# Vegeta2020/SE-SSD

Hardware: AMD Instinct MI355X
Metric: KITTI frames/sec (voxelize->backbone->head->NMS) (higher is better)
Workload: dtype f32

## Files before the change

### se-ssd_amd/csrc/dense_wino_sk.hip

```cpp
#include <cstdlib>
#include "common.hpp"
#include "bf16_split.hpp"

namespace {

using f32x16 = __attribute__((ext_vector_type(16))) float;
using f32x4v = __attribute__((ext_vector_type(4))) float;
using f32x2v = __attribute__((ext_vector_type(2))) float;
typedef unsigned int u32x4g __attribute__((__vector_size__(16)));
typedef __bf16 bf16x8 __attribute__((ext_vector_type(8)));
typedef __bf16 bf16x2 __attribute__((ext_vector_type(2)));

typedef __amdgpu_buffer_rsrc_t rsrc_t;
__device__ __forceinline__ rsrc_t make_rsrc(const void* base, unsigned bytes) {
  return __builtin_amdgcn_make_buffer_rsrc(const_cast<void*>(base), (short)0, (int)bytes, 0x00020000);
}
#define SESSD_OOB 0x80000000u
#define SESSD_LDS_BARRIER() asm volatile("s_waitcnt lgkmcnt(0)\n\ts_barrier" ::: "memory")
#define SESSD_SYSTEM_SCOPE 17

__device__ __forceinline__ float sadd(float a, float b) {
  float r;
  asm volatile("v_add_f32 %0, %1, %2" : "=v"(r) : "v"(a), "v"(b));
  return r;
}

using sessd::pk_bf16;
using sessd::split3_pk;

struct WinoArgs {
  const float* in;
  const float* upk;
  float* out;
  const float* scale;
  const float* shift;
  const float* residual;
  float* scratch;
  unsigned* counters;
  int cin, hin, win, cout, relu;
  int tw, ntiles, tblocks, ngroups, rpu, total_rounds;
  int bper;
  int ss_stride;
  long long upk_stride;
  const int* tile_list;
  const int* n_list;
  int list_cap, min_rounds, batch;
};

template <int NW, int CBN, int VAR = 0, bool LIST = false, bool SPLIT = false>
__global__ __launch_bounds__(NW * 64, 8 / NW) void conv3x3s1_winograd_sk_kernel(WinoArgs A) {
  constexpr int XW = 16 / NW;
  static_assert(XW * CBN == 8, "8 accumulators per wave");
  static_assert(!SPLIT || (NW == 8 && VAR == 0), "the split main loop is written for 8 waves (a round = one K = 16 MFMA)");
  constexpr int VBUF_S = 3 * 16 * 64 * 4;
  constexpr int NT = NW * 64;
  constexpr unsigned WSTEP = NW * 2u * 32u * 32u;
  constexpr int VBUF = NW * 1024;
  constexpr int SLOT = CBN * 32 * 32 * 4;
  constexpr int NPT = 1024 / NT;
  constexpr int RING = NW;
  __shared__ __attribute__((aligned(16))) float lds[SPLIT ? 2 * VBUF_S : 16384];
  __shared__ int s_last, s_pend;
  const int tid = threadIdx.x, lane = tid & 63;
  const int wave = __builtin_amdgcn_readfirstlane(tid >> 6);
  const int j = lane & 31, h = lane >> 5;
  int G = gridDim.x;
  long long R = A.total_rounds;
  int n_list = 0;
  if constexpr (LIST) {
    n_list = __builtin_amdgcn_readfirstlane(min(A.n_list[0], A.list_cap));
    R = (long long)((n_list + 31) >> 5) * A.ngroups * A.rpu;
    if (R == 0) return;
    if (A.min_rounds < 0) {
      const long long U = R / A.rpu;
      long long g = U / (-A.min_rounds);
      g = g < 1 ? 1 : (g > G ? G : g);
      G = (int)g;
      if ((int)blockIdx.x >= G) return;
    } else {
      long long g = R / A.min_rounds;
      g = g < 1 ? 1 : (g > G ? G : g);
      G = (int)(g >= 8 ? (g & ~7LL) : g);
      if ((G & 7) ? ((int)blockIdx.x >= G) : ((int)(blockIdx.x >> 3) >= (G >> 3))) return;
    }
  }
  const bool whole_units = LIST && A.min_rounds < 0;
  const int w = (whole_units || (G & 7)) ? (int)blockIdx.x : (int)((blockIdx.x & 7) * (G >> 3) + (blockIdx.x >> 3));
  int r = whole_units ? (int)((long long)w * (R / A.rpu) / G) * A.rpu : (int)((long long)w * R / G);
  const int r_stop = whole_units ? (int)((long long)(w + 1) * (R / A.rpu) / G) * A.rpu : (int)((long long)(w + 1) * R / G);
  const int in_plane = A.hin * A.win;
  const size_t out_plane = (size_t)in_plane;
  const unsigned xstep = 2u * (unsigned)in_plane * 4u;
  const unsigned wo = (unsigned)(((wave * 2 + h) * 32 + j) * 32);

  int pend_state = 0, pend_u = 0, pend_first = 0, pend_last = 0, pend_tbase = 0, pend_mbase = 0, pend_b = 0;
#define SESSD_SK_SIGNAL()                                                                          \
  {                                                                                                \
    __builtin_amdgcn_s_waitcnt(0);                                                                 \
    __syncthreads();                                                                               \
    if (tid == 0) {                                                                                \
      const unsigned old = __hip_atomic_fetch_add(A.counters + pend_u, 1u, __ATOMIC_RELAXED, __HIP_MEMORY_SCOPE_AGENT); \
      s_pend = (old == (unsigned)(pend_last - pend_first)) ? 1 : 0;                                \
    }                                                                                              \
    __syncthreads();                                                                               \
    pend_state = s_pend ? 2 : 0;                                                                   \
  }

#define SESSD_SK_FINALIZE(Y, CO, SC, SH)                                                            \
  if (tok && (CO) < e_cout) {                                                                       \
    _Pragma("unroll") for (int a = 0; a < 2; ++a) {                                                 \
      const size_t o = (size_t)(CO) * out_plane + pix + (size_t)a * e_win;                          \
      float v0 = fmaf((Y)[2 * a], (SC), (SH)), v1 = fmaf((Y)[2 * a + 1], (SC), (SH));              \
      if (e_relu) { v0 = fmaxf(v0, 0.f); v1 = fmaxf(v1, 0.f); }                                 \
      if (resb) { v0 += resb[o]; v1 += resb[o + 1]; }                                               \
      *reinterpret_cast<float2*>(outb + o) = make_float2(v0, v1);                                   \
    }                                                                                               \
  }
#define SESSD_SK_FINISH_PENDING()                                                                  \
  {                                                                                                \
    const __attribute__((address_space(4))) WinoArgs* Fp =                                         \
        (const __attribute__((address_space(4))) WinoArgs*)__builtin_amdgcn_kernarg_segment_ptr(); \
    asm volatile("" : "+s"(Fp));                                                                   \
    const int f_set = pend_b / Fp->bper;                                                           \
    const float* f_scale = Fp->scale ? Fp->scale + (size_t)f_set * Fp->ss_stride : nullptr;        \
    const float* f_shift = Fp->shift ? Fp->shift + (size_t)f_set * Fp->ss_stride : nullptr;        \
    const int e_cout = Fp->cout, e_relu = Fp->relu, e_win = Fp->win, f_tw = Fp->tw;                \
    const rsrc_t fr = make_rsrc(Fp->scratch, (unsigned)(2 * G) * SLOT * 4u);                       \
    float* outb = Fp->out + (size_t)pend_b * e_cout * out_plane;                                   \
    const float* resb = Fp->residual ? Fp->residual + (size_t)pend_b * e_cout * out_plane : nullptr; \
    const int tl = tid & 31, col0 = tid >> 5;                                                      \
    int tt = pend_tbase + tl;                                                                      \
    bool tok = tt < Fp->ntiles;                                                                    \
    size_t pix = 0;                                                                                \
    if constexpr (LIST) {                                                                          \
      const int fe = tt < n_list ? Fp->tile_list[tt] : -1;                                         \
      tok = fe >= 0;                                                                               \
      const int fb = tok ? fe / Fp->ntiles : 0;                                                    \
      tt = tok ? fe - fb * Fp->ntiles : 0;                                                         \
      pix = (size_t)fb * e_cout * out_plane;                                                       \
    }                                                                                              \
    const int oty = tok ? tt / f_tw : 0, otx = tok ? tt - (tt / f_tw) * f_tw : 0;                  \
    pix += (size_t)(2 * oty) * e_win + 2 * otx;                                                    \
    _Pragma("unroll 1") for (int cb = 0; cb < CBN; ++cb) {                                         \
      f32x4v ysum[NPT];                                                                            \
      _Pragma("unroll") for (int n = 0; n < NPT; ++n) ysum[n] = 0.f;                               \
      for (int wq = pend_first; wq <= pend_last; ++wq) {                                           \
        const unsigned slot = (unsigned)(2 * wq + (wq == pend_first ? 1 : 0)) * (unsigned)(SLOT * 4); \
        f32x4v p[NPT];                                                                             \
        _Pragma("unroll") for (int n = 0; n < NPT; ++n)                                            \
          p[n] = __builtin_bit_cast(f32x4v, __builtin_amdgcn_raw_buffer_load_b128(                 \
              fr, (int)(slot + (unsigned)(((cb * 32 + col0 + (NT / 32) * n) * 32 + tl) * 16)), 0, SESSD_SYSTEM_SCOPE)); \
        _Pragma("unroll") for (int n = 0; n < NPT; ++n) ysum[n] += p[n];                           \
      }                                                                                            \
      _Pragma("unroll") for (int n = 0; n < NPT; ++n) {                                            \
        const int co = pend_mbase + cb * 32 + col0 + (NT / 32) * n;                                \
        const float scv = (f_scale && co < e_cout) ? f_scale[co] : 1.f, shv = (f_shift && co < e_cout) ? f_shift[co] : 0.f; \
        const float z[4] = {ysum[n].x, ysum[n].y, ysum[n].z, ysum[n].w};                           \
        SESSD_SK_FINALIZE(z, co, scv, shv)                                                         \
      }                                                                                            \
    }                                                                                              \
    if (tid == 0) __hip_atomic_store(Fp->counters + pend_u, 0u, __ATOMIC_RELAXED, __HIP_MEMORY_SCOPE_AGENT); \
    pend_state = 0;                                                                                \
  }

  while (r < r_stop) {
    const int u = __builtin_amdgcn_readfirstlane(r / A.rpu);
    const int r0 = __builtin_amdgcn_readfirstlane(r - u * A.rpu);
    const int r1 = __builtin_amdgcn_readfirstlane(min(r_stop - u * A.rpu, A.rpu));
    r = u * A.rpu + r1;
    const int cg = __builtin_amdgcn_readfirstlane(u % A.ngroups), ub = u / A.ngroups;
    const int tb = LIST ? __builtin_amdgcn_readfirstlane(ub) : __builtin_amdgcn_readfirstlane(ub % A.tblocks);
    const int b = LIST ? 0 : __builtin_amdgcn_readfirstlane(ub / A.tblocks);
    const int t_base = tb * 32, m_base = cg * (CBN * 32);
    const rsrc_t xr = LIST ? make_rsrc(A.in, (unsigned)A.batch * (unsigned)A.cin * (unsigned)in_plane * 4u)
                           : make_rsrc(A.in + (size_t)b * A.cin * in_plane, (unsigned)A.cin * in_plane * 4u);
    const int wset = LIST ? 0 : __builtin_amdgcn_readfirstlane(b / A.bper);
    const rsrc_t wr = make_rsrc(A.upk + (size_t)wset * A.upk_stride + (size_t)cg * (A.cin >> 1) * (WSTEP / 4), (unsigned)(A.cin >> 1) * WSTEP);

    int t = t_base + j;
    bool tlive = t < A.ntiles;
    unsigned img_off = 0;
    if constexpr (LIST) {
      const int e = t < n_list ? A.tile_list[t] : -1;
      tlive = e >= 0;
      const int bl = tlive ? e / A.ntiles : 0;
      t = tlive ? e - bl * A.ntiles : 0;
      img_off = (unsigned)bl * (unsigned)A.cin * (unsigned)in_plane * 4u;
    }
    const int ty = tlive ? t / A.tw : 0, tx = tlive ? t - (t / A.tw) * A.tw : 0;
    const int y0 = 2 * ty - 1, x0 = 2 * tx - 1;
    unsigned ro[4];
#pragma unroll
    for (int q = 0; q < 4; ++q) {
      const int y = y0 + q;
      ro[q] = (tlive && y >= 0 && y < A.hin) ? img_off + (unsigned)((h * in_plane + y * A.win + max(x0, 0)) * 4) : SESSD_OOB;
    }
    const bool mask_l = (tx == 0), mask_r = (tx == A.tw - 1);
    const bool edge = __builtin_amdgcn_ballot_w64(tlive && (mask_l || mask_r)) != 0;
    const int klast = r1 * NW - 1;

    f32x16 acc[XW][CBN];
#pragma unroll
    for (int x = 0; x < XW; ++x)
#pragma unroll
      for (int c = 0; c < CBN; ++c)
#pragma unroll
// ... 30 lines not shown
#define SESSD_SK_TRANSFORM(VOFF)                                                                   \
  {                                                                                                \
    if (edge) {                                                                                    \
      _Pragma("unroll") for (int q = 0; q < 4; ++q) {                                              \
        const f32x4v p = pr[q];                                                                    \
        pr[q].x = mask_l ? 0.f : p.x; pr[q].y = mask_l ? p.x : p.y;                                \
        pr[q].z = mask_l ? p.y : p.z; pr[q].w = mask_l ? p.z : (mask_r ? 0.f : p.w);               \
      }                                                                                            \
    }                                                                                              \
    f32x2v tl[4], tr[4];                                                                           \
    if constexpr (VAR & 1) {                                                                       \
      tl[0].x = sadd(pr[0].x, -pr[2].x); tl[0].y = sadd(pr[0].y, -pr[2].y); tr[0].x = sadd(pr[0].z, -pr[2].z); tr[0].y = sadd(pr[0].w, -pr[2].w); \
      tl[1].x = sadd(pr[1].x, pr[2].x); tl[1].y = sadd(pr[1].y, pr[2].y); tr[1].x = sadd(pr[1].z, pr[2].z); tr[1].y = sadd(pr[1].w, pr[2].w); \
      tl[2].x = sadd(pr[2].x, -pr[1].x); tl[2].y = sadd(pr[2].y, -pr[1].y); tr[2].x = sadd(pr[2].z, -pr[1].z); tr[2].y = sadd(pr[2].w, -pr[1].w); \
      tl[3].x = sadd(pr[1].x, -pr[3].x); tl[3].y = sadd(pr[1].y, -pr[3].y); tr[3].x = sadd(pr[1].z, -pr[3].z); tr[3].y = sadd(pr[1].w, -pr[3].w); \
    } else {                                                                                       \
    tl[0] = pr[0].xy - pr[2].xy; tr[0] = pr[0].zw - pr[2].zw;                                      \
    tl[1] = pr[1].xy + pr[2].xy; tr[1] = pr[1].zw + pr[2].zw;                                      \
    tl[2] = pr[2].xy - pr[1].xy; tr[2] = pr[2].zw - pr[1].zw;                                      \
    tl[3] = pr[1].xy - pr[3].xy; tr[3] = pr[1].zw - pr[3].zw;                                      \
    }                                                                                              \
    float* dst = &lds[(VOFF) + wave * 1024 + h * 32 + j];                                          \
    _Pragma("unroll") for (int a = 0; a < 4; ++a) {                                                \
      dst[(a * 4 + 0) * 64] = tl[a].x - tr[a].x;                                                   \
      dst[(a * 4 + 1) * 64] = tl[a].y + tr[a].x;                                                   \
      dst[(a * 4 + 2) * 64] = tr[a].x - tl[a].y;                                                   \
      dst[(a * 4 + 3) * 64] = tl[a].y - tr[a].y;                                                   \
    }                                                                                              \
  }
#define SESSD_SK_READV(P, KS, VOFF)                                                                \
  {                                                                                                \
    const float* vb = &lds[(VOFF) + (KS)*1024 + wave * (XW * 64) + h * 32 + j];                    \
    _Pragma("unroll") for (int x = 0; x < XW; ++x) bv[P][x] = vb[x * 64];                          \
  }
#define SESSD_SK_MMA(SET, P)                                                                       \
  {                                                                                                \
    if constexpr (VAR & 2) __builtin_amdgcn_s_setprio(3);                                          \
    _Pragma("unroll") for (int c = 0; c < CBN; ++c)                                                \
      _Pragma("unroll") for (int x = 0; x < XW; ++x)                                               \
        acc[x][c] = __builtin_amdgcn_mfma_f32_32x32x2f32(ua[SET][(c * XW + x) >> 2][(c * XW + x) & 3], bv[P][x], acc[x][c], 0, 0, 0); \
    if constexpr (VAR & 2) __builtin_amdgcn_s_setprio(0);                                          \
  }
#define SESSD_SK_STEP(KS)                                                                          \
  {                                                                                                \
    SESSD_SK_LOADU(((KS) + RING - 1) & (RING - 1), kg0 + (KS) + RING - 1)                          \
    if ((KS) < NW - 1) SESSD_SK_READV(((KS) + 1) & 1, (KS) + 1, voff)                              \
    __builtin_amdgcn_sched_barrier(0);                                                             \
    SESSD_SK_MMA((KS) & (RING - 1), (KS) & 1)                                                      \
    __builtin_amdgcn_sched_barrier(0);                                                             \
  }
#define SESSD_SK_ROUND()                                                                           \
  {                                                                                                \
    const int kg0 = rr * NW;                                                                       \
    SESSD_SK_LOADP(rr + 1)                                                                         \
    SESSD_SK_READV(0, 0, voff)                                                                     \
    __builtin_amdgcn_sched_barrier(0);                                                             \
    SESSD_SK_STEP(0)                                                                               \
    SESSD_SK_STEP(1)                                                                               \
    SESSD_SK_STEP(2)                                                                               \
    SESSD_SK_STEP(3)                                                                               \
    if constexpr (NW == 8) {                                                                       \
      SESSD_SK_STEP(4)                                                                             \
      SESSD_SK_STEP(5)                                                                             \
      SESSD_SK_STEP(6)                                                                             \
      SESSD_SK_STEP(7)                                                                             \
    }                                                                                              \
    SESSD_SK_TRANSFORM(voff ^ VBUF)                                                                \
    __syncthreads();                                                                               \
    voff ^= VBUF;                                                                                  \
    ++rr;                                                                                          \
  }
#define SESSD_SS_LOADP(ROUND)                                                                      \
  {                                                                                                \
    const unsigned xs = (unsigned)(min((ROUND), r1 - 1) * NW + wave) * xstep;                      \
    _Pragma("unroll") for (int c = 0; c < 2; ++c)                                                  \
      _Pragma("unroll") for (int q = 0; q < 3; ++q)                                                \
        ps[c][q] = __builtin_bit_cast(f32x4v, __builtin_amdgcn_raw_buffer_load_b128(xr, (int)rs[q], (int)(xs + c * (xstep >> 1)), 0)); \
  }
#define SESSD_SS_LOADU(SET, KG)                                                                    \
  {                                                                                                \
    const unsigned ws = (unsigned)min((KG), klast) * 3072u;                                        \
    _Pragma("unroll") for (int p = 0; p < 3; ++p)                                                  \
      us[SET][p] = __builtin_bit_cast(bf16x8, __builtin_amdgcn_raw_buffer_load_b128(wrs, (int)(wso + 1024u * p), (int)ws, 0)); \
  }
#define SESSD_SS_TRANSFORM(VOFF)                                                                   \
  {                                                                                                \
    if (edge) {                                                                                    \
      _Pragma("unroll") for (int c = 0; c < 2; ++c)                                                \
        _Pragma("unroll") for (int q = 0; q < 3; ++q) {                                            \
          const f32x4v p = ps[c][q];                                                               \
          ps[c][q].x = mask_l ? 0.f : p.x; ps[c][q].y = mask_l ? p.x : p.y;                        \
          ps[c][q].z = mask_l ? p.y : p.z; ps[c][q].w = mask_l ? p.z : (mask_r ? 0.f : p.w);       \
        }                                                                                          \
    }                                                                                              \
    float vt[2][8];                                                                                \
    _Pragma("unroll") for (int c = 0; c < 2; ++c) {                                                \
      const f32x4v ra = ps[c][0] - ps[c][1];                                                       \
      const f32x4v rb = ps[c][1] + (h ? -ps[c][2] : ps[c][2]);                                     \
      vt[c][0] = ra.x - ra.z; vt[c][1] = ra.y + ra.z; vt[c][2] = ra.z - ra.y; vt[c][3] = ra.y - ra.w; \
      vt[c][4] = rb.x - rb.z; vt[c][5] = rb.y + rb.z; vt[c][6] = rb.z - rb.y; vt[c][7] = rb.y - rb.w; \
    }                                                                                              \
    unsigned* dst = reinterpret_cast<unsigned*>(&lds[(VOFF) + ((8 * h) * 64 + (wave >> 2) * 32 + j) * 4 + (wave & 3)]); \
    _Pragma("unroll") for (int e = 0; e < 8; ++e) {                                                \
      unsigned t0, t1, t2;                                                                         \
      split3_pk(vt[0][e], vt[1][e], t0, t1, t2);                                                   \
      dst[e * 256] = t0; dst[(16 + e) * 256] = t1; dst[(32 + e) * 256] = t2;                       \
    }                                                                                              \
  }
#define SESSD_SS_READV(VOFF, X)                                                                    \
  {                                                                                                \
    _Pragma("unroll") for (int p = 0; p < 3; ++p)                                                  \
      bs[p] = __builtin_bit_cast(bf16x8, *static_cast<const u32x4g*>(__builtin_assume_aligned(                    \
          &lds[(VOFF) + ((p * 16 + wave * XW + (X)) * 64 + lane) * 4], 16)));                     \
  }
#define SESSD_SS_MMA(SET, S)                                                                       \
  {                                                                                                \
    f32x16 a_ = acc[(S) >> 2][(S) & 3];                                                            \
    a_ = __builtin_amdgcn_mfma_f32_32x32x16_bf16(us[SET][2], bs[0], a_, 0, 0, 0);                  \
    a_ = __builtin_amdgcn_mfma_f32_32x32x16_bf16(us[SET][1], bs[1], a_, 0, 0, 0);                  \
    a_ = __builtin_amdgcn_mfma_f32_32x32x16_bf16(us[SET][0], bs[2], a_, 0, 0, 0);                  \
    a_ = __builtin_amdgcn_mfma_f32_32x32x16_bf16(us[SET][1], bs[0], a_, 0, 0, 0);                  \
    a_ = __builtin_amdgcn_mfma_f32_32x32x16_bf16(us[SET][0], bs[1], a_, 0, 0, 0);                  \
    a_ = __builtin_amdgcn_mfma_f32_32x32x16_bf16(us[SET][0], bs[0], a_, 0, 0, 0);                  \
    acc[(S) >> 2][(S) & 3] = a_;                                                                   \
  }
#define SESSD_SS_STEP(KS)                                                                          \
  {                                                                                                \
    SESSD_SS_LOADU(((KS) + 3) & 3, kg0 + (KS) + 3)                                                 \
    __builtin_amdgcn_sched_barrier(0);                                                             \
    SESSD_SS_MMA((KS) & 3, KS)                                                                     \
    __builtin_amdgcn_sched_barrier(0);                                                             \
  }
#define SESSD_SS_ROUND()                                                                           \
  {                                                                                                \
    const int kg0 = rr * 8;                                                                        \
    SESSD_SS_READV(voff, 0)                                                                        \
    __builtin_amdgcn_sched_barrier(0);                                                             \
    SESSD_SS_STEP(0)                                                                               \
    SESSD_SS_STEP(1)                                                                               \
    SESSD_SS_STEP(2)                                                                               \
    SESSD_SS_STEP(3)                                                                               \
    SESSD_SS_LOADP(rr + 1)                                                                         \
    SESSD_SS_READV(voff, 1)                                                                        \
    __builtin_amdgcn_sched_barrier(0);                                                             \
    SESSD_SS_STEP(4)                                                                               \
    SESSD_SS_STEP(5)                                                                               \
    SESSD_SS_STEP(6)                                                                               \
    SESSD_SS_STEP(7)                                                                               \
    SESSD_SS_TRANSFORM(voff ^ VBUF_S)                                                              \
    __syncthreads();                                                                               \
    voff ^= VBUF_S;                                                                                \
    ++rr;                                                                                          \
  }

    if constexpr (SPLIT) {
      SESSD_SS_LOADP(r0)
      __builtin_amdgcn_sched_barrier(0);
#pragma unroll
      for (int s = 0; s < 3; ++s) {
        SESSD_SS_LOADU(s, r0 * 8 + s)
        __builtin_amdgcn_sched_barrier(0);
      }
      SESSD_SS_TRANSFORM(0)
    } else {
      SESSD_SK_LOADP(r0)
      __builtin_amdgcn_sched_barrier(0);
#pragma unroll
      for (int s = 0; s < RING - 1; ++s) {
        SESSD_SK_LOADU(s, r0 * NW + s)
        __builtin_amdgcn_sched_barrier(0);
      }
      SESSD_SK_TRANSFORM(0)
    }
    __syncthreads();
    if (pend_state == 1) {
      if (tid == 0) {
        const unsigned old = __hip_atomic_fetch_add(A.counters + pend_u, 1u, __ATOMIC_RELAXED, __HIP_MEMORY_SCOPE_AGENT);
        s_pend = (old == (unsigned)(pend_last - pend_first)) ? 1 : 0;
      }
      pend_state = 3;
    }
    int voff = 0;
    int rr = r0;
    if constexpr (SPLIT) {
      while (rr < r1) SESSD_SS_ROUND()
    } else {
      while (rr < r1) SESSD_SK_ROUND()
    }
#undef SESSD_SK_LOADP
#undef SESSD_SK_LOADU
#undef SESSD_SK_TRANSFORM
#undef SESSD_SK_READV
#undef SESSD_SK_MMA
#undef SESSD_SK_STEP
#undef SESSD_SK_ROUND
#undef SESSD_SS_LOADP
#undef SESSD_SS_LOADU
#undef SESSD_SS_TRANSFORM
#undef SESSD_SS_READV
#undef SESSD_SS_MMA
#undef SESSD_SS_STEP
#undef SESSD_SS_ROUND

    if (pend_state == 3) {
      SESSD_LDS_BARRIER();
      pend_state = s_pend ? 2 : 0;
    }
    const __attribute__((address_space(4))) WinoArgs* Ep =
        (const __attribute__((address_space(4))) WinoArgs*)__builtin_amdgcn_kernarg_segment_ptr();
    asm volatile("" : "+s"(Ep));
    const float* e_scale = Ep->scale ? Ep->scale + (size_t)wset * Ep->ss_stride : nullptr;
    const float* e_shift = Ep->shift ? Ep->shift + (size_t)wset * Ep->ss_stride : nullptr;
    const int e_cout = Ep->cout, e_relu = Ep->relu, e_win = Ep->win, e_tw = Ep->tw, e_ntiles = Ep->ntiles;
    unsigned* e_counter = Ep->counters + u;
    const rsrc_t sr = make_rsrc(Ep->scratch, (unsigned)(2 * G) * SLOT * 4u);
    const bool full = (r0 == 0 && r1 == Ep->rpu);
    float* outb = Ep->out + (size_t)b * e_cout * out_plane;
    const float* resb = Ep->residual ? Ep->residual + (size_t)b * e_cout * out_plane : nullptr;
    const int tl = tid & 31, col0 = tid >> 5;
    int tt = t_base + tl;
    bool tok = tt < e_ntiles;
    size_t pix = 0;
    if constexpr (LIST) {
      const int ee = tt < n_list ? Ep->tile_list[tt] : -1;
      tok = ee >= 0;
      const int eb = tok ? ee / e_ntiles : 0;
      tt = tok ? ee - eb * e_ntiles : 0;
      pix = (size_t)eb * e_cout * out_plane;
    }
    const int oty = tok ? tt / e_tw : 0, otx = tok ? tt - (tt / e_tw) * e_tw : 0;
    pix += (size_t)(2 * oty) * e_win + 2 * otx;
    const int w_first = (int)((((long long)u * Ep->rpu + 1) * G - 1) / R);
    const int w_last = (int)((((long long)u * Ep->rpu + Ep->rpu) * G - 1) / R);
    const unsigned my_slot = (unsigned)(2 * w + (r0 == 0 ? 1 : 0)) * (unsigned)(SLOT * 4);
    bool certain = false;
    unsigned oslot = 0;
    if (!full && w_last == w_first + 1) {
      if (tid == 0) s_last = __hip_atomic_load(e_counter, __ATOMIC_RELAXED, __HIP_MEMORY_SCOPE_AGENT) == 1u ? 1 : 0;
      __syncthreads();
      certain = s_last != 0;
      const int wq = (w == w_first) ? w_last : w_first;
      oslot = (unsigned)(2 * wq + (wq == w_first ? 1 : 0)) * (unsigned)(SLOT * 4);
    }
    const bool writes_out = full || certain;
    f32x4v onext[NPT];
    float scn[NPT], shn[NPT];
#define SESSD_SK_FETCH(CB)                                                                          \
  _Pragma("unroll") for (int n = 0; n < NPT; ++n) {                                                 \
    const int co_ = m_base + (CB)*32 + col0 + (NT / 32) * n;                                        \
    if (certain)                                                                                    \
      onext[n] = __builtin_bit_cast(                                                                \
          f32x4v, __builtin_amdgcn_raw_buffer_load_b128(                                            \
                      sr, (int)(oslot + (unsigned)((((CB)*32 + col0 + (NT / 32) * n) * 32 + tl) * 16)), 0, SESSD_SYSTEM_SCOPE)); \
    else                                                                                            \
      onext[n] = 0.f;                                                                               \
    scn[n] = (writes_out && e_scale && co_ < e_cout) ? e_scale[co_] : 1.f;                          \
    shn[n] = (writes_out && e_shift && co_ < e_cout) ? e_shift[co_] : 0.f;                          \
  }
    SESSD_SK_FETCH(0)
#pragma unroll
    for (int cb = 0; cb < CBN; ++cb) {
      if (cb) SESSD_LDS_BARRIER();
#pragma unroll
      for (int x = 0; x < XW; ++x)
#pragma unroll
        for (int q = 0; q < 16; ++q) {
          const int co = (q & 3) + 8 * (q >> 2) + 4 * h;
          lds[((wave * XW + x) * 32 + co) * 32 + j] = acc[x][cb][q];
        }
      f32x4v other[NPT];
      float sc[NPT], sh[NPT];
#pragma unroll
      for (int n = 0; n < NPT; ++n) { other[n] = onext[n]; sc[n] = scn[n]; sh[n] = shn[n]; }
      if (cb + 1 < CBN) { SESSD_SK_FETCH(cb + 1) }
      SESSD_LDS_BARRIER();
#pragma unroll
      for (int n = 0; n < NPT; ++n) {
        const int col = col0 + (NT / 32) * n;
        float m[16];
#pragma unroll
        for (int x = 0; x < 16; ++x) m[x] = lds[(x * 32 + col) * 32 + tl];
        float q0[4], q1[4];
#pragma unroll
        for (int c = 0; c < 4; ++c) {
          q0[c] = m[0 * 4 + c] + m[1 * 4 + c] + m[2 * 4 + c];
          q1[c] = m[1 * 4 + c] - m[2 * 4 + c] - m[3 * 4 + c];
        }
        float y[4];
        y[0] = q0[0] + q0[1] + q0[2]; y[1] = q0[1] - q0[2] - q0[3];
        y[2] = q1[0] + q1[1] + q1[2]; y[3] = q1[1] - q1[2] - q1[3];
        const int co = m_base + cb * 32 + col;
        if (full) {
          SESSD_SK_FINALIZE(y, co, sc[n], sh[n])
        } else if (certain) {
          const f32x4v o4 = other[n];
          const bool mine_first = (w == w_first);
          float z[4];
          z[0] = mine_first ? (0.f + y[0]) + o4.x : (0.f + o4.x) + y[0];
          z[1] = mine_first ? (0.f + y[1]) + o4.y : (0.f + o4.y) + y[1];
          z[2] = mine_first ? (0.f + y[2]) + o4.z : (0.f + o4.z) + y[2];
          z[3] = mine_first ? (0.f + y[3]) + o4.w : (0.f + o4.w) + y[3];
          SESSD_SK_FINALIZE(z, co, sc[n], sh[n])
        } else {
          f32x4v v;
          v.x = y[0]; v.y = y[1]; v.z = y[2]; v.w = y[3];
          __builtin_amdgcn_raw_buffer_store_b128(__builtin_bit_cast(u32x4g, v), sr,
                                                 (int)(my_slot + (unsigned)(((cb * 32 + col) * 32 + tl) * 16)), 0, SESSD_SYSTEM_SCOPE);
        }
      }
    }
    if (certain) {
      if (tid == 0) __hip_atomic_store(e_counter, 0u, __ATOMIC_RELAXED, __HIP_MEMORY_SCOPE_AGENT);
    } else if (!full) {
      if (pend_state == 2) SESSD_SK_FINISH_PENDING()
      pend_u = u; pend_first = w_first; pend_last = w_last; pend_tbase = t_base; pend_mbase = m_base; pend_b = b;
      pend_state = 1;
    }
#undef SESSD_SK_FETCH
    SESSD_LDS_BARRIER();
  }
  if (pend_state == 1) SESSD_SK_SIGNAL()
  if (pend_state == 2) SESSD_SK_FINISH_PENDING()
#undef SESSD_SK_FINALIZE
#undef SESSD_SK_SIGNAL
#undef SESSD_SK_FINISH_PENDING
}


template <int VAR = 0>
__global__ __launch_bounds__(256, 1) void conv3x3s1_winograd_rk_kernel(WinoArgs A) {
  constexpr int NW = 4, KR = 8, RING = 4;
  constexpr int NT = NW * 64;
  constexpr unsigned WSTEP = 4u * 2u * 32u * 16u * 4u;
  constexpr int VBUF = KR * 1024;
  constexpr int SLOT = 4 * 32 * 32 * 4;
  constexpr int NPT = 1024 / NT;
  __shared__ __attribute__((aligned(16))) float lds[2 * VBUF];
  __shared__ int s_last, s_pend;
  const int tid = threadIdx.x, lane = tid & 63;
  const int wave = __builtin_amdgcn_readfirstlane(tid >> 6);
  const int j = lane & 31, h = lane >> 5;
  const int G = gridDim.x;
  const int w = (G & 7) ? (int)blockIdx.x : (int)((blockIdx.x & 7) * (G >> 3) + (blockIdx.x >> 3));
  const long long R = A.total_rounds;
  int r = (int)((long long)w * R / G);
  const int r_stop = (int)((long long)(w + 1) * R / G);
  const int in_plane = A.hin * A.win;
  const size_t out_plane = (size_t)in_plane;
  const unsigned xstep = 2u * (unsigned)in_plane * 4u;
  const unsigned wo = (unsigned)(((wave * 2 + h) * 32 + j) * 64);

  int pend_state = 0, pend_u = 0, pend_first = 0, pend_last = 0, pend_tbase = 0, pend_mbase = 0, pend_b = 0;
#define SESSD_RK_SIGNAL()                                                                          \
  {                                                                                                \
    __builtin_amdgcn_s_waitcnt(0);                                                                 \
// ... 192 lines not shown
#undef SESSD_RK_READV
#undef SESSD_RK_MMA
#undef SESSD_RK_STEP
#undef SESSD_RK_ROUND

    if (pend_state == 3) {
      SESSD_LDS_BARRIER();
      pend_state = s_pend ? 2 : 0;
    }
    const __attribute__((address_space(4))) WinoArgs* Ep =
        (const __attribute__((address_space(4))) WinoArgs*)__builtin_amdgcn_kernarg_segment_ptr();
    asm volatile("" : "+s"(Ep));
    const float* e_scale = Ep->scale ? Ep->scale + (size_t)wset * Ep->ss_stride : nullptr;
    const float* e_shift = Ep->shift ? Ep->shift + (size_t)wset * Ep->ss_stride : nullptr;
    const int e_cout = Ep->cout, e_relu = Ep->relu, e_win = Ep->win, e_tw = Ep->tw, e_ntiles = Ep->ntiles;
    unsigned* e_counter = Ep->counters + u;
    const rsrc_t sr = make_rsrc(Ep->scratch, (unsigned)(2 * G) * SLOT * 4u);
    const bool full = (r0 == 0 && r1 == Ep->rpu);
    float* outb = Ep->out + (size_t)b * e_cout * out_plane;
    const float* resb = Ep->residual ? Ep->residual + (size_t)b * e_cout * out_plane : nullptr;
    const int tt = t_base + j;
    const bool tok = tt < e_ntiles;
    const int oty = tok ? tt / e_tw : 0, otx = tok ? tt - (tt / e_tw) * e_tw : 0;
    const size_t pix = (size_t)(2 * oty) * e_win + 2 * otx;
    const int w_first = (int)((((long long)u * Ep->rpu + 1) * G - 1) / R);
    const int w_last = (int)((((long long)u * Ep->rpu + Ep->rpu) * G - 1) / R);
    const unsigned my_slot = (unsigned)(2 * w + (r0 == 0 ? 1 : 0)) * (unsigned)(SLOT * 4);
    bool certain = false;
    unsigned oslot = 0;
    if (!full && w_last == w_first + 1) {
      if (tid == 0) s_last = __hip_atomic_load(e_counter, __ATOMIC_RELAXED, __HIP_MEMORY_SCOPE_AGENT) == 1u ? 1 : 0;
      __syncthreads();
      certain = s_last != 0;
      const int wq = (w == w_first) ? w_last : w_first;
      oslot = (unsigned)(2 * wq + (wq == w_first ? 1 : 0)) * (unsigned)(SLOT * 4);
    }
    const bool writes_out = full || certain;
    const int col_base = wave * 32 + 4 * h;
#pragma unroll
    for (int half = 0; half < 2; ++half) {
      float sc[8], sh[8];
      f32x4v other[8];
#pragma unroll
      for (int e = 0; e < 8; ++e) {
        const int q = half * 8 + e;
        const int col = col_base + (q & 3) + 8 * (q >> 2);
        const int co_ = m_base + col;
        sc[e] = (writes_out && e_scale && co_ < e_cout) ? e_scale[co_] : 1.f;
        sh[e] = (writes_out && e_shift && co_ < e_cout) ? e_shift[co_] : 0.f;
        if (certain)
          other[e] = __builtin_bit_cast(f32x4v, __builtin_amdgcn_raw_buffer_load_b128(
                                                    sr, (int)(oslot + (unsigned)((col * 32 + j) * 16)), 0, SESSD_SYSTEM_SCOPE));
        else
          other[e] = 0.f;
      }
#pragma unroll
      for (int e = 0; e < 8; ++e) {
        const int q = half * 8 + e;
        const int col = col_base + (q & 3) + 8 * (q >> 2);
        float q0[4], q1[4];
#pragma unroll
        for (int c = 0; c < 4; ++c) {
          q0[c] = acc[0 * 4 + c][q] + acc[1 * 4 + c][q] + acc[2 * 4 + c][q];
          q1[c] = acc[1 * 4 + c][q] - acc[2 * 4 + c][q] - acc[3 * 4 + c][q];
        }
        float y[4];
        y[0] = q0[0] + q0[1] + q0[2]; y[1] = q0[1] - q0[2] - q0[3];
        y[2] = q1[0] + q1[1] + q1[2]; y[3] = q1[1] - q1[2] - q1[3];
        const int co = m_base + col;
        if (full) {
          SESSD_RK_FINALIZE(y, co, sc[e], sh[e])
        } else if (certain) {
          const f32x4v o4 = other[e];
          const bool mine_first = (w == w_first);
          float z[4];
          z[0] = mine_first ? (0.f + y[0]) + o4.x : (0.f + o4.x) + y[0];
          z[1] = mine_first ? (0.f + y[1]) + o4.y : (0.f + o4.y) + y[1];
          z[2] = mine_first ? (0.f + y[2]) + o4.z : (0.f + o4.z) + y[2];
          z[3] = mine_first ? (0.f + y[3]) + o4.w : (0.f + o4.w) + y[3];
          SESSD_RK_FINALIZE(z, co, sc[e], sh[e])
        } else {
          f32x4v v;
          v.x = y[0]; v.y = y[1]; v.z = y[2]; v.w = y[3];
          __builtin_amdgcn_raw_buffer_store_b128(__builtin_bit_cast(u32x4g, v), sr, (int)(my_slot + (unsigned)((col * 32 + j) * 16)), 0,
                                                 SESSD_SYSTEM_SCOPE);
        }
      }
    }
    if (certain) {
      if (tid == 0) __hip_atomic_store(e_counter, 0u, __ATOMIC_RELAXED, __HIP_MEMORY_SCOPE_AGENT);
    } else if (!full) {
      if (pend_state == 2) SESSD_RK_FINISH_PENDING()
      pend_u = u; pend_first = w_first; pend_last = w_last; pend_tbase = t_base; pend_mbase = m_base; pend_b = b;
      pend_state = 1;
    }
  }
  if (pend_state == 1) SESSD_RK_SIGNAL()
  if (pend_state == 2) SESSD_RK_FINISH_PENDING()
#undef SESSD_RK_FINALIZE
#undef SESSD_RK_SIGNAL
#undef SESSD_RK_FINISH_PENDING
}

int launch_rk(const float* in, int batch, int nsets, int cin, int h, int w, const float* upk, float* out, int cout, const float* scale,
              const float* shift, int relu, const float* residual, void* workspace, size_t workspace_bytes, int workgroups,
              hipStream_t stream) {
  constexpr int SLOT = 4 * 32 * 32 * 4;
  if (cin % 16) return SESSD_EINVAL;
  WinoArgs A;
  A.in = in; A.upk = upk; A.out = out; A.scale = scale; A.shift = shift; A.residual = residual;
  A.cin = cin; A.hin = h; A.win = w; A.cout = cout; A.relu = relu;
  A.tw = w / 2; A.ntiles = (h / 2) * (w / 2); A.tblocks = sessd_divup(A.ntiles, 32); A.ngroups = sessd_divup(cout, 128);
  A.rpu = cin / 16;
  A.bper = batch / nsets; A.ss_stride = nsets > 1 ? cout : 0;
  A.upk_stride = nsets > 1 ? (long long)sessd_divup(cout, 128) * (cin >> 1) * (4 * 2 * 32 * 16) : 0;
  A.tile_list = nullptr; A.n_list = nullptr; A.list_cap = 0; A.min_rounds = 1; A.batch = batch;
  const long long units = (long long)batch * A.tblocks * A.ngroups;
  if (units * A.rpu > 0x7fffffffLL) return SESSD_EINVAL;
  A.total_rounds = (int)(units * A.rpu);
  const size_t need = sessd_align((size_t)units * 4, 256) + (size_t)2 * workgroups * SLOT * 4;
  if (need > workspace_bytes) return SESSD_EWORKSPACE;
  if (workgroups > A.total_rounds) workgroups = A.total_rounds >= 8 ? (A.total_rounds & ~7) : A.total_rounds;
  A.counters = (unsigned*)workspace;
  A.scratch = (float*)((char*)workspace + sessd_align((size_t)units * 4, 256));
  SESSD_LAUNCH((conv3x3s1_winograd_rk_kernel<0>), dim3(workgroups), dim3(256), 0, stream, A);
  SESSD_CHECK_LAUNCH();
  return SESSD_OK;
}

template <int NW, int CBN, bool SPLIT = false>
int launch_sk(const float* in, int batch, int nsets, int cin, int h, int w, const float* upk, float* out, int cout, const float* scale,
              const float* shift, int relu, const float* residual, void* workspace, size_t workspace_bytes, int workgroups,
              hipStream_t stream, const int* tile_list = nullptr, const int* n_list = nullptr, int list_cap = 0, int min_rounds = 1) {
  constexpr int SLOT = CBN * 32 * 32 * 4;
  if (cin % (2 * NW)) return SESSD_EINVAL;
  if (tile_list && (nsets != 1 || !n_list || list_cap < 1 || (size_t)batch * cin * h * w * 4 >= 0xFFFFFFFFull)) return SESSD_EINVAL;
  WinoArgs A;
  A.in = in; A.upk = upk; A.out = out; A.scale = scale; A.shift = shift; A.residual = residual;
  A.cin = cin; A.hin = h; A.win = w; A.cout = cout; A.relu = relu;
  A.tw = w / 2; A.ntiles = (h / 2) * (w / 2); A.tblocks = sessd_divup(A.ntiles, 32); A.ngroups = sessd_divup(cout, CBN * 32);
  A.rpu = cin / (2 * NW);
  A.bper = batch / nsets; A.ss_stride = nsets > 1 ? cout : 0;
  A.upk_stride = nsets > 1 ? (long long)sessd_divup(cout, CBN * 32) * (cin >> 1) * (NW * 2 * 32 * 32 / 4) : 0;
  if (SPLIT && nsets > 1) A.upk_stride = (long long)sessd_divup(cout, CBN * 32) * cin * 3072;
  A.tile_list = tile_list; A.n_list = n_list; A.list_cap = list_cap; A.min_rounds = (min_rounds < 0 && tile_list) ? min_rounds : (min_rounds < 1 ? 1 : min_rounds); A.batch = batch;
  const long long units = (long long)batch * A.tblocks * A.ngroups;
  if (units * A.rpu > 0x7fffffffLL) return SESSD_EINVAL;
  A.total_rounds = (int)(units * A.rpu);
  const size_t need = sessd_align((size_t)units * 4, 256) + (size_t)2 * workgroups * SLOT * 4;
  if (need > workspace_bytes) return SESSD_EWORKSPACE;
  if (workgroups > A.total_rounds) workgroups = A.total_rounds >= 8 ? (A.total_rounds & ~7) : A.total_rounds;
  A.counters = (unsigned*)workspace;
  A.scratch = (float*)((char*)workspace + sessd_align((size_t)units * 4, 256));
  if (tile_list) {
    SESSD_LAUNCH((conv3x3s1_winograd_sk_kernel<NW, CBN, 0, true, SPLIT>), dim3(workgroups), dim3(NW * 64), 0, stream, A);
    SESSD_CHECK_LAUNCH();
    return SESSD_OK;
  }
  if constexpr (SPLIT) {
    SESSD_LAUNCH((conv3x3s1_winograd_sk_kernel<NW, CBN, 0, false, true>), dim3(workgroups), dim3(NW * 64), 0, stream, A);
    SESSD_CHECK_LAUNCH();
    return SESSD_OK;
  }
  static const int var = [] { const char* e = getenv("SESSD_WINO_VAR"); return e ? atoi(e) & 3 : 0; }();
  switch (var) {
    case 1: SESSD_LAUNCH((conv3x3s1_winograd_sk_kernel<NW, CBN, 1>), dim3(workgroups), dim3(NW * 64), 0, stream, A); break;
    case 2: SESSD_LAUNCH((conv3x3s1_winograd_sk_kernel<NW, CBN, 2>), dim3(workgroups), dim3(NW * 64), 0, stream, A); break;
    case 3: SESSD_LAUNCH((conv3x3s1_winograd_sk_kernel<NW, CBN, 3>), dim3(workgroups), dim3(NW * 64), 0, stream, A); break;
    default: SESSD_LAUNCH((conv3x3s1_winograd_sk_kernel<NW, CBN, 0>), dim3(workgroups), dim3(NW * 64), 0, stream, A); break;
  }
  SESSD_CHECK_LAUNCH();
  return SESSD_OK;
}

int default_workgroups(int shape, int* out) {
  int dev = 0, cus = 0;
  SESSD_TRY(hipGetDevice(&dev));
  SESSD_TRY(hipDeviceGetAttribute(&cus, hipDeviceAttributeMultiprocessorCount, dev));
  *out = ((shape == 1 ? 2 : 1) * cus) & ~7;
  return *out >= 8 ? SESSD_OK : SESSD_EINVAL;
}

}

extern "C" {

size_t sessd_conv3x3_winograd_sk_workspace_bytes(int batch, int h, int w, int cout, int shape, int workgroups) {
  if (batch < 1 || h < 2 || w < 2 || cout < 1 || workgroups < 0 || shape < 0 || shape > 3) return 0;
  if (workgroups == 0 && default_workgroups(shape, &workgroups) != SESSD_OK) return 0;
  const int cpu = shape == 1 ? 64 : 128;
  const size_t units = (size_t)batch * sessd_divup((h / 2) * (w / 2), 32) * sessd_divup(cout, cpu);
  return sessd_align(units * 4, 256) + (size_t)2 * workgroups * (cpu * 32 * 4) * 4;
}

int sessd_conv3x3_winograd_sk_sets(const float* in, int batch, int nsets, int cin, int h, int w, const float* upk, float* out,
                                   int cout, const float* scale, const float* shift, int relu, const float* residual,
                                   void* workspace, size_t workspace_bytes, int shape, int workgroups, hipStream_t stream) {
  if ((h & 1) || (w & 1) || batch < 1 || nsets < 1 || batch % nsets || cout < 1 || workgroups < 0 || (workgroups & 7) || shape < 0 ||
      shape > 3)
    return SESSD_EINVAL;
  if (workgroups == 0) {
    const int rc = default_workgroups(shape, &workgroups);
    if (rc != SESSD_OK) return rc;
  }
  if (shape == 2)
    return launch_rk(in, batch, nsets, cin, h, w, upk, out, cout, scale, shift, relu, residual, workspace, workspace_bytes, workgroups, stream);
  if (shape == 1)
    return launch_sk<4, 2>(in, batch, nsets, cin, h, w, upk, out, cout, scale, shift, relu, residual, workspace, workspace_bytes, workgroups, stream);
  if (shape == 3)
    return launch_sk<8, 4, true>(in, batch, nsets, cin, h, w, upk, out, cout, scale, shift, relu, residual, workspace, workspace_bytes, workgroups, stream);
  return launch_sk<8, 4>(in, batch, nsets, cin, h, w, upk, out, cout, scale, shift, relu, residual, workspace, workspace_bytes, workgroups, stream);
}

int sessd_conv3x3_winograd_sk_active(const float* in, int batch, int cin, int h, int w, const float* upk, float* out, int cout,
                                     const float* scale, const float* shift, int relu, const float* residual,
                                     const int32_t* tile_list, const int32_t* n_list, int list_cap, int min_rounds, void* workspace,
                                     size_t workspace_bytes, int shape, int workgroups, hipStream_t stream) {
  if ((h & 1) || (w & 1) || batch < 1 || cout < 1 || workgroups < 0 || (workgroups & 7) || shape < 0 || shape > 3 || shape == 2 ||
      !tile_list || !n_list || list_cap < 1)
    return SESSD_EINVAL;
  if (workgroups == 0) {
    const int rc = default_workgroups(shape, &workgroups);
    if (rc != SESSD_OK) return rc;
  }
  if (shape == 1)
    return launch_sk<4, 2>(in, batch, 1, cin, h, w, upk, out, cout, scale, shift, relu, residual, workspace, workspace_bytes, workgroups,
                           stream, tile_list, n_list, list_cap, min_rounds);
  if (shape == 3)
    return launch_sk<8, 4, true>(in, batch, 1, cin, h, w, upk, out, cout, scale, shift, relu, residual, workspace, workspace_bytes,
                                 workgroups, stream, tile_list, n_list, list_cap, min_rounds);
  return launch_sk<8, 4>(in, batch, 1, cin, h, w, upk, out, cout, scale, shift, relu, residual, workspace, workspace_bytes, workgroups,
                         stream, tile_list, n_list, list_cap, min_rounds);
}

int sessd_conv3x3_winograd_sk(const float* in, int batch, int cin, int h, int w, const float* upk, float* out, int cout,
                              const float* scale, const float* shift, int relu, const float* residual, void* workspace,
                              size_t workspace_bytes, int shape, int workgroups, hipStream_t stream) {
  return sessd_conv3x3_winograd_sk_sets(in, batch, 1, cin, h, w, upk, out, cout, scale, shift, relu, residual, workspace,
                                        workspace_bytes, shape, workgroups, stream);
}

}
```

Before: 2288.

## Interleave Winograd input transform with MFMA steps in split main loop

In the split (bf16x3) Winograd main loop, the per-round input tile transform and the 3-term bf16 split are broken into small fragments. These fragments are placed between the six MFMAs of steps 3–7 using sched_barriers, where they previously ran as one block after the MFMAs. The aim is to hide the VALU transform and LDS store work behind matrix-core execution. The old serialized loop stays reachable through variant bit 2 of SESSD_WINO_VAR, and the launch dispatch is reorganized to pick between them. This adds register pressure and leaves the fixed manual schedule more fragile.

```diff
diff --git a/se-ssd_amd/csrc/dense_wino_sk.hip b/se-ssd_amd/csrc/dense_wino_sk.hip
--- a/se-ssd_amd/csrc/dense_wino_sk.hip
+++ b/se-ssd_amd/csrc/dense_wino_sk.hip
@@ -22,6 +22,16 @@
 __device__ __forceinline__ float sadd(float a, float b) {
   float r;
   asm volatile("v_add_f32 %0, %1, %2" : "=v"(r) : "v"(a), "v"(b));
+  return r;
+}
+__device__ __forceinline__ float ssub(float a, float b) {
+  float r;
+  asm volatile("v_sub_f32 %0, %1, %2" : "=v"(r) : "v"(a), "v"(b));
+  return r;
+}
+__device__ __forceinline__ float sfma(float a, float b, float c) {
+  float r;
+  asm volatile("v_fma_f32 %0, %1, %2, %3" : "=v"(r) : "v"(a), "v"(b), "v"(c));
   return r;
 }
 
@@ -51,7 +61,8 @@
 __global__ __launch_bounds__(NW * 64, 8 / NW) void conv3x3s1_winograd_sk_kernel(WinoArgs A) {
   constexpr int XW = 16 / NW;
   static_assert(XW * CBN == 8, "8 accumulators per wave");
-  static_assert(!SPLIT || (NW == 8 && VAR == 0), "the split main loop is written for 8 waves (a round = one K = 16 MFMA)");
+  static_assert(!SPLIT || (NW == 8 && (VAR & 3) == 0), "the split main loop is written for 8 waves (a round = one K = 16 MFMA)");
+  static_assert(SPLIT || (VAR & 4) == 0, "variant bit 2 belongs to the split main loop");
   constexpr int VBUF_S = 3 * 16 * 64 * 4;
   constexpr int NT = NW * 64;
   constexpr unsigned WSTEP = NW * 2u * 32u * 32u;
@@ -388,6 +399,88 @@
     voff ^= VBUF_S;                                                                                \
     ++rr;                                                                                          \
   }
+#define SESSD_SS_F_MASK(R, C)                                                                      \
+  {                                                                                                \
+    const f32x4v p = R[C];                                                                         \
+    R[C].x = mask_l ? 0.f : p.x; R[C].y = mask_l ? p.x : p.y;                                      \
+    R[C].z = mask_l ? p.y : p.z; R[C].w = mask_l ? p.z : (mask_r ? 0.f : p.w);                     \
+  }
+#define SESSD_SS_F_ROWA(C)                                                                         \
+  {                                                                                                \
+    ra[C].x = ssub(ps[C][0].x, ps[C][1].x); ra[C].y = ssub(ps[C][0].y, ps[C][1].y);                \
+    ra[C].z = ssub(ps[C][0].z, ps[C][1].z); ra[C].w = ssub(ps[C][0].w, ps[C][1].w);                \
+  }
+#define SESSD_SS_F_ROWB(C)                                                                         \
+  {                                                                                                \
+    rb[C].x = sfma(ps[C][2].x, sgn, ps[C][1].x); rb[C].y = sfma(ps[C][2].y, sgn, ps[C][1].y);      \
+    rb[C].z = sfma(ps[C][2].z, sgn, ps[C][1].z); rb[C].w = sfma(ps[C][2].w, sgn, ps[C][1].w);      \
+  }
+#define SESSD_SS_F_COLS(C, R, O)                                                                   \
+  {                                                                                                \
+    vt[C][(O) + 0] = ssub(R[C].x, R[C].z); vt[C][(O) + 1] = sadd(R[C].y, R[C].z);                  \
+    vt[C][(O) + 2] = ssub(R[C].z, R[C].y); vt[C][(O) + 3] = ssub(R[C].y, R[C].w);                  \
+  }
+#define SESSD_SS_F_TERM(T, E)                                                                      \
+  {                                                                                                \
+    T = pk_bf16(vt[0][E], vt[1][E]);                                                               \
+    vt[0][E] = ssub(vt[0][E], __builtin_bit_cast(float, T << 16));                                 \
+    vt[1][E] = ssub(vt[1][E], __builtin_bit_cast(float, T & 0xFFFF0000u));                         \
+  }
+#define SESSD_SS_F_E0(E) SESSD_SS_F_TERM(tq0, E)
+#define SESSD_SS_F_E1(E) SESSD_SS_F_TERM(tq1, E)
+#define SESSD_SS_F_E2(E)                                                                           \
+  {                                                                                                \
+    vdst[(E) * 256] = tq0; vdst[(16 + (E)) * 256] = tq1; vdst[(32 + (E)) * 256] = pk_bf16(vt[0][E], vt[1][E]); \
+  }
+#define SESSD_SS_GAP(F)                                                                            \
+  __builtin_amdgcn_sched_barrier(0);                                                               \
+  F                                                                                                \
+  __builtin_amdgcn_sched_barrier(0);
+#define SESSD_SS_STEP_T(KS, F0, F1, F2, F3, F4, F5)                                                \
+  {                                                                                                \
+    SESSD_SS_LOADU(((KS) + 3) & 3, kg0 + (KS) + 3)                                                 \
+    __builtin_amdgcn_sched_barrier(0);                                                             \
+    f32x16 a_ = acc[(KS) >> 2][(KS) & 3];                                                          \
+    a_ = __builtin_amdgcn_mfma_f32_32x32x16_bf16(us[(KS) & 3][2], bs[0], a_, 0, 0, 0);             \
+    SESSD_SS_GAP(F0)                                                                               \
+    a_ = __builtin_amdgcn_mfma_f32_32x32x16_bf16(us[(KS) & 3][1], bs[1], a_, 0, 0, 0);             \
+    SESSD_SS_GAP(F1)                                                                               \
+    a_ = __builtin_amdgcn_mfma_f32_32x32x16_bf16(us[(KS) & 3][0], bs[2], a_, 0, 0, 0);             \
+    SESSD_SS_GAP(F2)                                                                               \
+    a_ = __builtin_amdgcn_mfma_f32_32x32x16_bf16(us[(KS) & 3][1], bs[0], a_, 0, 0, 0);             \
+    SESSD_SS_GAP(F3)                                                                               \
+    a_ = __builtin_amdgcn_mfma_f32_32x32x16_bf16(us[(KS) & 3][0], bs[1], a_, 0, 0, 0);             \
+    SESSD_SS_GAP(F4)                                                                               \
+    a_ = __builtin_amdgcn_mfma_f32_32x32x16_bf16(us[(KS) & 3][0], bs[0], a_, 0, 0, 0);             \
+    SESSD_SS_GAP(F5)                                                                               \
+    acc[(KS) >> 2][(KS) & 3] = a_;                                                                 \
+  }
+#define SESSD_SS_ROUND_PIPE()                                                                      \
+  {                                                                                                \
+    const int kg0 = rr * 8;                                                                        \
+    f32x4v ra[2], rb[2];                                                                           \
+    float vt[2][8];                                                                                \
+    unsigned tq0, tq1;                                                                             \
+    unsigned* vdst = reinterpret_cast<unsigned*>(&lds[(voff ^ VBUF_S) + ((8 * h) * 64 + (wave >> 2) * 32 + j) * 4 + (wave & 3)]); \
+    SESSD_SS_LOADP(rr + 1)                                                                         \
+    SESSD_SS_READV(voff, 0)                                                                        \
+    __builtin_amdgcn_sched_barrier(0);                                                             \
+    SESSD_SS_STEP(0)                                                                               \
+    SESSD_SS_STEP(1)                                                                               \
+    SESSD_SS_STEP(2)                                                                               \
+    SESSD_SS_STEP_T(3, SESSD_SS_F_ROWA(0) SESSD_SS_F_ROWA(1), SESSD_SS_F_ROWB(0) SESSD_SS_F_ROWB(1), SESSD_SS_F_MASK(ra, 0),    \
+                    SESSD_SS_F_MASK(ra, 1), SESSD_SS_F_MASK(rb, 0), SESSD_SS_F_MASK(rb, 1))        \
+    SESSD_SS_READV(voff, 1)                                                                        \
+    __builtin_amdgcn_sched_barrier(0);                                                             \
+    SESSD_SS_STEP_T(4, SESSD_SS_F_COLS(0, ra, 0) SESSD_SS_F_COLS(1, ra, 0), SESSD_SS_F_E0(0), SESSD_SS_F_E1(0),              \
+                    SESSD_SS_F_E2(0) SESSD_SS_F_COLS(0, rb, 4), SESSD_SS_F_E0(1) SESSD_SS_F_COLS(1, rb, 4), SESSD_SS_F_E1(1)) \
+    SESSD_SS_STEP_T(5, SESSD_SS_F_E2(1) SESSD_SS_F_E0(2), SESSD_SS_F_E1(2), SESSD_SS_F_E2(2), SESSD_SS_F_E0(3), SESSD_SS_F_E1(3), SESSD_SS_F_E2(3)) \
+    SESSD_SS_STEP_T(6, SESSD_SS_F_E0(4), SESSD_SS_F_E1(4), SESSD_SS_F_E2(4), SESSD_SS_F_E0(5), SESSD_SS_F_E1(5), SESSD_SS_F_E2(5)) \
+    SESSD_SS_STEP_T(7, SESSD_SS_F_E0(6), SESSD_SS_F_E1(6), SESSD_SS_F_E2(6), SESSD_SS_F_E0(7), SESSD_SS_F_E1(7), SESSD_SS_F_E2(7)) \
+    __syncthreads();                                                                               \
+    voff ^= VBUF_S;                                                                                \
+    ++rr;                                                                                          \
+  }
 
     if constexpr (SPLIT) {
       SESSD_SS_LOADP(r0)
@@ -418,8 +511,11 @@
     }
     int voff = 0;
     int rr = r0;
-    if constexpr (SPLIT) {
+    if constexpr (SPLIT && (VAR & 4)) {
       while (rr < r1) SESSD_SS_ROUND()
+    } else if constexpr (SPLIT) {
+      const float sgn = h ? -1.f : 1.f;
+      while (rr < r1) SESSD_SS_ROUND_PIPE()
     } else {
       while (rr < r1) SESSD_SK_ROUND()
     }
@@ -437,6 +533,17 @@
 #undef SESSD_SS_MMA
 #undef SESSD_SS_STEP
 #undef SESSD_SS_ROUND
+#undef SESSD_SS_F_MASK
+#undef SESSD_SS_F_ROWA
+#undef SESSD_SS_F_ROWB
+#undef SESSD_SS_F_COLS
+#undef SESSD_SS_F_TERM
+#undef SESSD_SS_F_E0
+#undef SESSD_SS_F_E1
+#undef SESSD_SS_F_E2
+#undef SESSD_SS_GAP
+#undef SESSD_SS_STEP_T
+#undef SESSD_SS_ROUND_PIPE
 
     if (pend_state == 3) {
       SESSD_LDS_BARRIER();
@@ -935,18 +1042,24 @@
   if (workgroups > A.total_rounds) workgroups = A.total_rounds >= 8 ? (A.total_rounds & ~7) : A.total_rounds;
   A.counters = (unsigned*)workspace;
   A.scratch = (float*)((char*)workspace + sessd_align((size_t)units * 4, 256));
-  if (tile_list) {
-    SESSD_LAUNCH((conv3x3s1_winograd_sk_kernel<NW, CBN, 0, true, SPLIT>), dim3(workgroups), dim3(NW * 64), 0, stream, A);
+  static const int var = [] { const char* e = getenv("SESSD_WINO_VAR"); return e ? atoi(e) & 7 : 0; }();
+  if constexpr (SPLIT) {
+    if (tile_list) {
+      if (var & 4) SESSD_LAUNCH((conv3x3s1_winograd_sk_kernel<NW, CBN, 4, true, true>), dim3(workgroups), dim3(NW * 64), 0, stream, A);
+      else SESSD_LAUNCH((conv3x3s1_winograd_sk_kernel<NW, CBN, 0, true, true>), dim3(workgroups), dim3(NW * 64), 0, stream, A);
+    } else {
+      if (var & 4) SESSD_LAUNCH((conv3x3s1_winograd_sk_kernel<NW, CBN, 4, false, true>), dim3(workgroups), dim3(NW * 64), 0, stream, A);
+      else SESSD_LAUNCH((conv3x3s1_winograd_sk_kernel<NW, CBN, 0, false, true>), dim3(workgroups), dim3(NW * 64), 0, stream, A);
+    }
     SESSD_CHECK_LAUNCH();
     return SESSD_OK;
   }
-  if constexpr (SPLIT) {
-    SESSD_LAUNCH((conv3x3s1_winograd_sk_kernel<NW, CBN, 0, false, true>), dim3(workgroups), dim3(NW * 64), 0, stream, A);
+  if (tile_list) {
+    SESSD_LAUNCH((conv3x3s1_winograd_sk_kernel<NW, CBN, 0, true, false>), dim3(workgroups), dim3(NW * 64), 0, stream, A);
     SESSD_CHECK_LAUNCH();
     return SESSD_OK;
   }
-  static const int var = [] { const char* e = getenv("SESSD_WINO_VAR"); return e ? atoi(e) & 3 : 0; }();
-  switch (var) {
+  switch (var & 3) {
     case 1: SESSD_LAUNCH((conv3x3s1_winograd_sk_kernel<NW, CBN, 1>), dim3(workgroups), dim3(NW * 64), 0, stream, A); break;
     case 2: SESSD_LAUNCH((conv3x3s1_winograd_sk_kernel<NW, CBN, 2>), dim3(workgroups), dim3(NW * 64), 0, stream, A); break;
     case 3: SESSD_LAUNCH((conv3x3s1_winograd_sk_kernel<NW, CBN, 3>), dim3(workgroups), dim3(NW * 64), 0, stream, A); break;
```

Result: faster. 2330, median of 6 (+1.8%).
